# mit-acl/roman

Hardware: AMD Instinct MI355X
Metric: submap-pair alignments/sec + p50 latency at n=m=200 objects, d=512 (higher is better)
Workload: dtype f64 (fixed-point SpMV sums); 1 GPU; config 3: batch of 256 submap pairs per GPU, n=200 m=200 d=512, method=semanticgrav (xyz + 512-d descriptors + gravity prior); p50 latency measured on config 2 (single pair); pairs_per_call=256, n=200, m=200, d=512, method=semanticgrav, batches_in_flight=3

## Files before the change

roman_amd/csrc/kernels.hip.h:

```cpp
#pragma once
#include <hip/hip_cooperative_groups.h>
#include <hip/hip_runtime.h>
#include <stdint.h>
#include <type_traits>
#include "../../include/roman_hip.h"

namespace roman {

constexpr int WAVE = 64;
constexpr int STREAM_MAXL = 3072;

struct DevParams {
    roman_params_t p;
    double sig2;
    double sin_unc;
    double x_eps;
    double x_mindist;
    int32_t single;
    int32_t gravity;
    int32_t F;
    int32_t max_compact;
    int32_t gmode;
    int32_t diag_one;
    int32_t keep_all;
// ... 2266 lines not shown
        for (int t = 0; t < nw; ++t) { if (t < w) wbase += wsum[t]; tot += wsum[t]; }
        const uint32_t carry = carry_s;
        if (s < nsl) sliceBase[lo + s] = carry + wbase + inc - v;
        __syncthreads();
        if (tid == 0) carry_s = carry + tot;
        __syncthreads();
    }
    if (tid == 0) st[b].nnzCap = carry_s;
}

struct LivePools { int32_t* lp; int32_t* li; int32_t* lj; double* ls; double* ld; double* lza; double* lzb; };

__global__ void __launch_bounds__(1024) k_upper(const ProbDesc* __restrict__ probs, const ProbState* __restrict__ st,
                                                const BatchTotals* __restrict__ tot, const ItemDesc* __restrict__ items,
                                                const unsigned long long* __restrict__ maskPool,
                                                uint16_t* __restrict__ listPool, const uint32_t* __restrict__ listOff,
                                                uint32_t* __restrict__ rowCnt, const uint32_t* __restrict__ perm,
                                                const uint32_t* __restrict__ rowPos, LivePools src, LivePools dst, int RPB)
{
    __shared__ uint16_t posS[STREAM_MAXL + 64];
    const int tid = threadIdx.x, nt = blockDim.x, lane = tid & 63, w = tid >> 6, wpb = nt >> 6;
    const int nItems = tot->items;
    int staged = -1;
    const int Gx_ = (nItems + 7) >> 3;
    for (int sIdx_ = blockIdx.x; (sIdx_ >> 3) < Gx_; sIdx_ += gridDim.x) {
        const int t = (sIdx_ & 7) * Gx_ + (sIdx_ >> 3);
        if (t >= nItems) continue;
        const ItemDesc it = items[t];
        const int b = it.b;
        if (uni_i(st[b].kind) == 0) {
        const int L = st[b].L;
        const int W = (L + 63) >> 6;
        const int64_t lo = probs[b].liveOff, mo = st[b].maskOff;
        uint16_t* const lists = listPool + st[b].listOff;
        const int nrows = min(RPB, L - it.row0);
        if (staged != b) {
            __syncthreads();
            for (int q = tid; q < W * 64; q += nt) posS[q] = (q < L) ? (uint16_t)rowPos[lo + q] : (uint16_t)0;
            __syncthreads();
            staged = b;
        }
        const int RW = (nrows + wpb - 1) / wpb;
        const int r0 = w * RW, r1 = min(nrows, r0 + RW);
        if (r0 < r1) {
            const int p0 = it.row0 + r0;
            uint32_t glo = 0u, ghi = 0u;
            for (int wd = 0; wd < W; ++wd) {
                const unsigned long long gt = __ballot((int)posS[(wd << 6) + lane] > p0);
                writelane2(glo, ghi, gt, (uint32_t)__builtin_amdgcn_readfirstlane(wd));
            }
            unsigned long long behind = ((unsigned long long)ghi << 32) | glo;
            const int nr = r1 - r0;
            const int kv = (lane < nr) ? (int)perm[lo + p0 + lane] : 0;
            const uint32_t ov = (lane < nr) ? listOff[lo + p0 + lane] : 0u;
            if (lane < nr) { dst.lp[lo + p0 + lane] = src.lp[lo + kv]; dst.ld[lo + p0 + lane] = src.ld[lo + kv]; }
            unsigned long long m_n = (lane < W) ? maskPool[mo + (int64_t)__builtin_amdgcn_readlane(kv, 0) * W + lane] : 0ull;
            for (int i = 0; i < nr; ++i) {
                const int p = p0 + i;
                const unsigned long long raw = m_n;
                int kn = 0;
                if (i + 1 < nr) {
                    kn = __builtin_amdgcn_readlane(kv, i + 1);
                    m_n = (lane < W) ? maskPool[mo + (int64_t)kn * W + lane] : 0ull;
                }
                const unsigned long long mine = raw & behind;
                const uint32_t c = (uint32_t)__popcll(mine);
                const uint32_t ex = wave_excl_scan(c, lane);
                const uint32_t cnt = (uint32_t)__builtin_amdgcn_readlane((int)(ex + c), WAVE - 1);
                {
                    uint16_t* lst = lists + (uint32_t)__builtin_amdgcn_readlane((int)ov, i);
                    unsigned long long m = mine; uint32_t e = ex;
                    while (m) { lst[e++] = (uint16_t)((lane << 6) + __builtin_ctzll(m)); m &= m - 1ull; }
                    if (lane < 4 && cnt + (uint32_t)lane < ((cnt + 3u) & ~3u)) lst[cnt + lane] = (uint16_t)0xffffu;
                }
                if (lane == 0) rowCnt[lo + p] = cnt;
                if (i + 1 < nr && lane == (kn >> 6)) behind &= ~(1ull << (kn & 63));
            }
        }
        }
    }
}

constexpr int LISTS_NT = 1024;

__global__ void __launch_bounds__(LISTS_NT) k_lists(int B, const ProbDesc* __restrict__ probs, ProbState* __restrict__ st, BatchTotals* __restrict__ tot,
                                                   const unsigned long long* __restrict__ maskPool,
                                                   uint16_t* __restrict__ listPool, uint32_t* __restrict__ listOff,
                                                   uint32_t* __restrict__ rowCnt, uint32_t* __restrict__ perm, uint32_t* __restrict__ rowPos,
                                                   LivePools src, LivePools dst, long long capList,
                                                   int eqMax ,
                                                   int degGiven )
{
    __shared__ uint32_t degS[STREAM_MAXL + 64];
    __shared__ uint32_t keyS[4096];
    __shared__ unsigned long long tabS[STREAM_MAXL + 64];
    __shared__ uint16_t tmpS[STREAM_MAXL + 64];
    __shared__ uint32_t wsum[LISTS_NT / 64 + 4];
    __shared__ int okS;
    static_assert(STREAM_MAXL <= 4096, "sort capacity");
    const int tid = threadIdx.x, lane = tid & 63, w = tid >> 6;
    constexpr int NW = LISTS_NT / 64;
    const int g = lane >> 4, sl = lane & 15;
    for (int b = blockIdx.x; b < B; b += gridDim.x) {
        __syncthreads();
        if (st[b].kind != 0) continue;
        const int L = st[b].L;
        if (L <= 0) continue;
        const int W = (L + 63) >> 6;
        const int64_t lo = probs[b].liveOff, mo = st[b].maskOff;
        const unsigned long long* mrow = maskPool + mo;
        auto fetch = [&](int k0_, int c0_) -> unsigned long long {
            const int k = k0_ + g, c = c0_ + sl;
            const bool valid = k < L && c < W;
            unsigned long long m = mrow[(int64_t)min(k, L - 1) * W + min(c, W - 1)];
            if (!valid) m = 0ull;
            if (c == (k >> 6)) m &= ((k & 63) == 63) ? 0ull : (~0ull << ((k & 63) + 1));
            return m;
        };
        auto advance = [&](int& k0_, int& c0_) { c0_ += 16; if (c0_ >= W) { k0_ += 4 * NW; c0_ = k0_ >> 6; } };
        auto sweep = [&](auto f) {
            constexpr int PF = 6;
            int kr[PF], cr[PF]; unsigned long long mr[PF];
            int kn = 4 * w, cn = kn >> 6;
#pragma unroll
            for (int i = 0; i < PF; ++i) { kr[i] = kn; cr[i] = cn; mr[i] = fetch(kn, cn); advance(kn, cn); }
            while (kr[0] < L) {
#pragma unroll
                for (int i = 0; i < PF; ++i) {
                    const int kc = kr[i], cc = cr[i]; const unsigned long long mc = mr[i];
                    kr[i] = kn; cr[i] = cn; mr[i] = fetch(kn, cn); advance(kn, cn);
                    f(kc + g, mc, cc + sl);
                }
            }
        };
#ifdef ROMAN_LISTS_TIMING
        unsigned long long tl_[6]; tl_[0] = __builtin_readcyclecounter();
#define LMARK(i_) tl_[i_] = __builtin_readcyclecounter()
#else
#define LMARK(i_) do { } while (0)
#endif
        for (int q = tid; q < L; q += LISTS_NT) degS[q] = degGiven ? rowCnt[lo + q] : 0u;
        __syncthreads();
        if (!degGiven) {
        sweep([&](int k, unsigned long long m, int c) {
            if (m) {
                atomicAdd(&degS[k], (uint32_t)__popcll(m));
                while (m) { atomicAdd(&degS[(c << 6) + __builtin_ctzll(m)], 1u); m &= m - 1ull; }
            }
        });
        __syncthreads();
        }
        LMARK(1);
        int N = 64; while (N < L) N <<= 1;
        if (eqMax <= 0 || !place_keys(L, N, eqMax, [&](int k) { return degS[k]; }, keyS, reinterpret_cast<uint32_t*>(tabS), reinterpret_cast<uint32_t*>(tabS) + (STREAM_MAXL + 64), tmpS, wsum)) {
        for (int t = tid; t < N; t += LISTS_NT) keyS[t] = (t < L) ? (((degS[t] + 1u) << 12) | (uint32_t)(4095 - t)) : 0u;
        __syncthreads();
        for (int k2 = 2; k2 <= N; k2 <<= 1)
            for (int j2 = k2 >> 1; j2 > 0; j2 >>= 1) {
                for (int t = tid; t < (N >> 1); t += LISTS_NT) {
                    const int i1 = ((t & ~(j2 - 1)) << 1) | (t & (j2 - 1)), i2 = i1 | j2;
                    const uint32_t a = keyS[i1], c2 = keyS[i2];
                    const bool desc = (i1 & k2) == 0;
                    if ((a < c2) == desc) { keyS[i1] = c2; keyS[i2] = a; }
                }
                __syncthreads();
            }
        }
        LMARK(2);
        {
            const int PER = (L + LISTS_NT - 1) / LISTS_NT;
            uint32_t sum = 0;
            for (int t = 0; t < PER; ++t) {
                const int q = tid * PER + t;
                if (q < L) sum += (min((keyS[q] >> 12) - 1u, (uint32_t)(L - 1 - q)) + 3u) & ~3u;
            }
            const uint32_t inc = wave_incl_scan(sum);
            if (lane == WAVE - 1) wsum[w] = inc;
            __syncthreads();
            uint32_t wbase = 0, total = 0;
            for (int t = 0; t < NW; ++t) { if (t < w) wbase += wsum[t]; total += wsum[t]; }
            if (tid == 0) {
                const unsigned long long base = atomicAdd(&tot->listTop, (unsigned long long)total);
                st[b].listOff = (int64_t)base;
                const bool fits = (long long)(base + total) <= capList;
                if (!fits) { st[b].kind = 2; atomicAdd(&tot->overflow, 1); }
                okS = fits ? 1 : 0;
            }
            uint32_t run = wbase + inc - sum;
            for (int t = 0; t < PER; ++t) {
                const int q = tid * PER + t;
                if (q < L) {
                    const uint32_t k = 4095u - (keyS[q] & 4095u);
                    perm[lo + q] = k; rowPos[lo + k] = (uint32_t)q;
                    tabS[k] = ((unsigned long long)run << 16) | (unsigned long long)q; listOff[lo + q] = run; degS[k] = 0u;
                    run += (min((keyS[q] >> 12) - 1u, (uint32_t)(L - 1 - q)) + 3u) & ~3u;
                }
            }
        }
        __syncthreads();
        if (!okS) continue;
        uint16_t* const lists = listPool + st[b].listOff;
        LMARK(3);
        sweep([&](int k, unsigned long long m, int c) {
            if (!m) return;
            const unsigned long long tk = tabS[k];
            const uint32_t pk = (uint32_t)tk & 0xffffu, ok = (uint32_t)(tk >> 16);
            while (m) {
                const uint32_t q = (uint32_t)((c << 6) + __builtin_ctzll(m));
                m &= m - 1ull;
                const unsigned long long tq = tabS[q];
                const bool mine = pk < ((uint32_t)tq & 0xffffu);
                const uint32_t slot = atomicAdd(&degS[mine ? (uint32_t)k : q], 1u);
                lists[(mine ? ok : (uint32_t)(tq >> 16)) + slot] = (uint16_t)(mine ? q : (uint32_t)k);
            }
        });
        __syncthreads();
        LMARK(4);
        for (int p = tid; p < L; p += LISTS_NT) {
            const uint32_t k = 4095u - (keyS[p] & 4095u);
            const uint32_t cnt = degS[k];
            rowCnt[lo + p] = cnt;
            uint16_t* lst = lists + (uint32_t)(tabS[k] >> 16);
            for (uint32_t e = cnt; e < ((cnt + 3u) & ~3u); ++e) lst[e] = (uint16_t)0xffffu;
            dst.lp[lo + p] = src.lp[lo + k]; dst.ld[lo + p] = src.ld[lo + k];
        }
#ifdef ROMAN_LISTS_TIMING
        LMARK(5);
        if (tid == 0 && (b & 63) == 0) printf("[k_lists] b=%d L=%d cycles: degrees %llu sort %llu offsets %llu scatter %llu tail %llu\n", b, L,
                                              tl_[1] - tl_[0], tl_[2] - tl_[1], tl_[3] - tl_[2], tl_[4] - tl_[3], tl_[5] - tl_[4]);
#endif
#undef LMARK
    }
}

__global__ void __launch_bounds__(64) k_slicegeom(const ProbDesc* __restrict__ probs, ProbState* __restrict__ st,
                                                  const uint32_t* __restrict__ rowCnt,
                                                  uint32_t* __restrict__ sliceWidth, uint32_t* __restrict__ sliceBase)
{
    const int b = blockIdx.x, lane = threadIdx.x;
    if (st[b].kind != 0) return;
    const int L = st[b].L;
    const int64_t lo = probs[b].liveOff;
    const int nsl = (L + 63) >> 6;
    uint32_t width = 0;
    if (lane < nsl) {
        const int hi = min(L, (lane << 6) + 64);
        for (int p = lane << 6; p < hi; ++p) width = max(width, rowCnt[lo + p]);
        width = (width + 3u) & ~3u;
        sliceWidth[lo + lane] = width;
    }
    const uint32_t v = width * 64u;
    const uint32_t ex = wave_excl_scan(v, lane);
    if (lane < nsl) sliceBase[lo + lane] = ex;
    if (lane == WAVE - 1) st[b].nnzCap = ex + v;
}

__global__ void __launch_bounds__(1024) k_probscan(int B, int NG , long long capNnz, ProbState* __restrict__ st, BatchTotals* __restrict__ tot)
{
    __shared__ long long shl[17];
    __shared__ int shi[17];
    __shared__ int red[1];
    const int tid = threadIdx.x, nt = blockDim.x;
    const int PER = (B + nt - 1) / nt;
    const int b0 = tid * PER, b1 = min(B, b0 + PER);
    constexpr int PC = 8;
    int cK[PC], cL[PC]; uint32_t cC[PC];
#pragma unroll
    for (int j = 0; j < PC; ++j) { const int b = b0 + j; const bool in = j < PER && b < b1; cK[j] = in ? st[b].kind : 2; cL[j] = in ? st[b].L : 0; cC[j] = in ? st[b].nnzCap : 0u; }
    auto get = [&](int b, int& kind, int& L, long long& cap) {
        const int j = b - b0;
        if (j < PC) {
#pragma unroll
            for (int t = 0; t < PC; ++t) if (t == j) { kind = cK[t]; L = cL[t]; cap = (long long)cC[t]; }
        } else { kind = st[b].kind; L = st[b].L; cap = (long long)st[b].nnzCap; }
        if (kind >= 2) cap = 0;
    };
    long long sC = 0;
    for (int b = b0; b < b1; ++b) { int kind, L; long long cap; get(b, kind, L, cap); sC += cap; }
    long long totC; int totG;
    const long long baseC = block_excl_scan(sC, shl, totC);
    int sG = 0;
    {
        long long acc = baseC;
        for (int b = b0; b < b1; ++b) {
            int kind, L; long long cap; get(b, kind, L, cap);
            acc += cap;
            if (kind == 0 && acc <= capNnz) sG += min(NG, (L + 63) >> 6);
        }
    }
    const int baseG = block_excl_scan(sG, shi, totG);
    if (tid == 0) red[0] = 0;
    __syncthreads();
    int nover = 0;
    {
        long long acc = baseC; int gacc = baseG;
        for (int b = b0; b < b1; ++b) {
            int kind, L; long long cap; get(b, kind, L, cap);
            const bool fits = acc + cap <= capNnz;
            const int ng = (kind == 0 && fits) ? min(NG, (L + 63) >> 6) : 0;
            st[b].nnzOff = fits ? acc : 0; st[b].sgBase = gacc;
            if (!fits && kind < 2) { st[b].kind = 2; ++nover; }
            acc += cap; gacc += ng;
        }
    }
    for (int off = 32; off > 0; off >>= 1) nover += __shfl_xor(nover, off);
    if ((tid & 63) == 0 && nover) atomicAdd(&red[0], nover);
    __syncthreads();
// ... 3159 lines not shown
```

roman_amd/csrc/roman_hip.hip:

```cpp
#include <hip/hip_runtime.h>
#include <algorithm>
#include <cmath>
#include <cstdarg>
#include <cstdio>
#include <cstdlib>
#include <cstring>
#include <new>
#include <string>
#include <vector>

#include "kernels.hip.h"

using namespace roman;

namespace {

thread_local std::string g_last_error;

struct DevBuf {
    void* p = nullptr; size_t cap = 0;
    hipError_t ensure(size_t bytes) {
        if (bytes <= cap) return hipSuccess;
        if (p) { hipError_t e = hipFree(p); p = nullptr; cap = 0; if (e != hipSuccess) return e; }
        size_t want = bytes + bytes / 4 + 256;
// ... 202 lines not shown
}
struct StageTimer {
    roman_ctx* c; int s;
    StageTimer(roman_ctx* c_, int s_) : c(c_), s(s_) { if (c->profile) { prof_flush(c, c->cur, s); (void)hipEventRecord(WS.evA[s], WS.stream); } }
    void stop() { if (c->profile) { (void)hipEventRecord(WS.evB[s], WS.stream); WS.pending[s] = true; } }
};

int dbg_stage(roman_ctx* c, const char* what)
{
    static const bool dbg = getenv("ROMAN_DEBUG") != nullptr;
    if (!dbg) return ROMAN_OK;
    const hipError_t e = hipStreamSynchronize(WS.stream);
    fprintf(stderr, "[roman] %-14s %s\n", what, e == hipSuccess ? "ok" : hipGetErrorString(e));
    fflush(stderr);
    return e == hipSuccess ? ROMAN_OK : fail(c, ROMAN_E_HIP, "%s failed: %s", what, hipGetErrorString(e));
}
#define DBG(c, what) do { int rc_ = dbg_stage((c), (what)); if (rc_) return rc_; } while (0)

struct BatchIn {
    int32_t B; const double* feats; const int64_t* off1; const int32_t* n1; const int64_t* off2; const int32_t* n2;
    int32_t F; const int32_t* assoc; const int64_t* assoc_off;
};

struct Sizing {
    double sumA = 0, maxA = 0, maskBound = 0;
    int expectMaxL = 0;
    long long capMaskWords = 0, capNnz = 0, capList = 0;
};

void harvest_totals(roman_ctx* c, bool wait)
{
    for (int k = 0; k < ROMAN_MAX_PIPELINE; ++k) {
        roman_ctx::Workspace& W = c->ws[k];
        if (!W.totPending || !W.totEvent) continue;
        if (wait) { if (hipEventSynchronize(W.totEvent) != hipSuccess) { (void)hipGetLastError(); continue; } }
        else if (hipEventQuery(W.totEvent) != hipSuccess) { (void)hipGetLastError(); continue; }
        W.totPending = false;
        const BatchTotals& t = *W.pinnedTotals;
        c->skippedTotal += t.overflow;
        if (W.totEpoch != c->histEpoch) continue;
        roman_ctx::Hist& H = c->hist;
        if (W.totMaxA > 0) H.rMaxL = std::max(H.rMaxL, (double)t.maxL / W.totMaxA);
        if (W.totMaskBound > 0) H.rMask = std::max(H.rMask, (double)t.needMaskWords / W.totMaskBound);
        if (W.totSumA > 0) H.rNnz = std::max(H.rNnz, (double)t.needNnz / W.totSumA);
        if (W.totSumA > 0) H.rList = std::max(H.rList, (double)t.listTop / W.totSumA);
        if (t.minStreamL <= SMALL_MAXL) H.smallSeen = true;
        if (t.maxStreamL > SMALL_MAXL) H.largeSeen = true;
        if (t.nGeneral > 0) H.generalSeen = true;
        if (t.cosScreened > 0) { H.cosSeen = true; H.cosDenseFrac = (double)t.cosDense / t.cosScreened; }
        H.valid = true;
    }
}

void estimate_sizes(roman_ctx* c, const DevParams& D, const roman_params_t* params, int32_t F, const std::vector<ProbDesc>& hd, Sizing* S)
{
    roman_ctx::Hist& H = c->hist;
    if (!H.tagged || H.F != F || memcmp(&H.params, params, sizeof(roman_params_t)) != 0) {
        H = roman_ctx::Hist{}; H.params = *params; H.F = F; H.tagged = true;
        ++c->histEpoch;
    }
    harvest_totals(c, false);
    const bool prunes = D.single && !D.keep_all;
    double heurMask = 0, heurNnz = 0; int heurMaxL = 0;
    for (const ProbDesc& d : hd) {
        const double nA = d.nA;
        S->sumA += nA; S->maxA = std::max(S->maxA, nA); S->maskBound += nA * std::ceil(nA / 64.0);
        const double capL = prunes ? std::min(nA, std::max(4096.0, nA / 8.0)) : nA;
        heurMaxL = std::max(heurMaxL, (int)capL);
        heurMask += capL * std::ceil(capL / 64.0);
        heurNnz += capL * std::min(capL, 96.0);
    }
    if (H.valid) {
        S->expectMaxL = prunes ? (int)std::min(S->maxA, std::ceil(H.rMaxL * S->maxA * 1.15) + 64.0) : (int)S->maxA;
        S->capMaskWords = (long long)(prunes ? H.rMask * S->maskBound * 1.3 + 4096.0 : S->maskBound);
        S->capNnz = (long long)(H.rNnz * S->sumA * 1.3 + 65536.0);
        S->capList = (long long)(H.rList * S->sumA * 1.3 + 65536.0);
    } else {
        S->expectMaxL = heurMaxL; S->capMaskWords = (long long)heurMask; S->capNnz = (long long)heurNnz + 65536;
        S->capList = (long long)(2.5 * heurNnz) + 65536;
    }
    S->capMaskWords = std::max<long long>(S->capMaskWords, 64);
    const char* tcap = getenv("ROMAN_TEST_CAPNNZ");
    if (tcap && !H.valid) S->capNnz = atoll(tcap);
}

int may_fallback(const DevParams& D, const std::vector<ProbDesc>& hd);

struct BatchOut { int32_t kmax; int32_t* assoc_out; int32_t* n_assoc_out; double* T_out; int32_t* status_out; roman_stats_t* stats_out; };

int make_solve_out(roman_ctx* c, int B, int64_t sumA, const BatchOut& out, SolveOut* O)
{
    const size_t R1 = (size_t)std::max<int64_t>(sumA, 1);
    HIPCHK(c, WS.uOut.ensure(sizeof(double) * R1)); HIPCHK(c, WS.nodesOrig.ensure(sizeof(int32_t) * R1));
    HIPCHK(c, WS.nSel.ensure(sizeof(int32_t) * (size_t)B));
    O->assoc_out = out.assoc_out; O->n_assoc_out = out.n_assoc_out; O->T_out = out.T_out; O->status_out = out.status_out; O->stats_out = out.stats_out; O->kmax = out.kmax;
    O->nodesOrig = WS.nodesOrig.as<int32_t>(); O->nSel = WS.nSel.as<int32_t>(); O->uOut = WS.uOut.as<double>();
    O->dbg = nullptr;
    return ROMAN_OK;
}

static hipError_t launch_cos_flagged(roman_ctx* c, hipStream_t stream, const DevParams& D, int B, int maxN1, int maxN2, const ProbDesc* dP, const double* feats,
                                     double* cosPool, const int32_t* dense);
static hipError_t launch_cos_sel(roman_ctx* c, hipStream_t stream, const DevParams& D, int B, int maxN1, int maxN2, const ProbDesc* dP, const double* feats, double* cosPool,
                                 int32_t* dense, bool approx)
{
    hipError_t e = dyn_lds(c, reinterpret_cast<const void*>(k_cos_sel), (size_t)CSEL_LDS);
    if (e != hipSuccess) return e;
    const double thr = approx ? INFINITY : D.p.cosine_min - 0x1p-6;
    hipLaunchKernelGGL(k_cos_sel, dim3((unsigned)B), dim3(1024), (size_t)CSEL_LDS, stream, D, B, dP, feats, cosPool, dense, thr);
    e = hipGetLastError();
    if (e != hipSuccess) return e;
    return launch_cos_flagged(c, stream, D, B, maxN1, maxN2, dP, feats, cosPool, dense);
}
static hipError_t launch_cos_live(roman_ctx* c, hipStream_t stream, const DevParams& D, int B, int maxN1, int maxN2, const ProbDesc* dP, const double* feats, double* cosPool,
                                  int32_t* dense, ProbState* st, const LivePools& LP)
{
    hipError_t e = dyn_lds(c, reinterpret_cast<const void*>(k_cos_live), (size_t)CSEL_LDS);
    if (e != hipSuccess) return e;
    hipLaunchKernelGGL(k_cos_live, dim3((unsigned)B), dim3(1024), (size_t)CSEL_LDS, stream, D, B, dP, feats, dense, D.p.cosine_min - 0x1p-6,
                       st, LP.lp, LP.li, LP.lj, LP.ls, LP.ld, LP.lza, LP.lzb);
    e = hipGetLastError();
    if (e != hipSuccess) return e;
    return launch_cos_flagged(c, stream, D, B, maxN1, maxN2, dP, feats, cosPool, dense);
}
static hipError_t launch_cos_flagged(roman_ctx* c, hipStream_t stream, const DevParams& D, int B, int maxN1, int maxN2, const ProbDesc* dP, const double* feats,
                                     double* cosPool, const int32_t* dense)
{
    hipError_t e;
    constexpr int TD = 5;
    using CD = CosDeal<TD>;
    const int Gd = CD::tiles(maxN1) * CD::tiles(maxN2);
    e = dyn_lds(c, reinterpret_cast<const void*>(k_cos_deal<TD, 0>), (size_t)CD::LDS);
    if (e != hipSuccess) return e;
    hipLaunchKernelGGL((k_cos_deal<TD, 0>), dim3((unsigned)(B >= 8 ? Gd * ((B + 7) / 8) * 8 : Gd * B)), dim3(256), (size_t)CD::LDS, stream, D, B, Gd, dP, feats, cosPool, (const int32_t*)dense);
    return hipGetLastError();
}
static bool cos_sel_applies(const roman_ctx* c, const DevParams& D, int B, int maxN1, int maxN2, int64_t poolRows)
{
    if (!D.single || D.pruned || !(D.p.cosine_max > D.p.cosine_min) || !std::isfinite(D.p.cosine_min) || !std::isfinite(D.p.cosine_max)) return false;
    if (maxN1 > CSEL_MAXN || maxN2 > CSEL_MAXN || maxN1 <= 0 || maxN2 <= 0) return false;
    if (poolRows * (int64_t)D.F * 8 >= (1LL << 32)) return false;
    const char* env = getenv("ROMAN_COS_SEL");
    if (env && env[0]) return env[0] == '1';
    if (2 * B < c->num_cu || D.p.cos_feature_dim < 64 || std::max(maxN1, maxN2) < 64) return false;
    roman_ctx::Hist& H = const_cast<roman_ctx*>(c)->hist;
    if (H.cosSeen && H.cosDenseFrac > 0.25) {
        if (++H.cosSkipped < 64) return false;
        H.cosSkipped = 0;
    }
    return true;
}


static int sort_eq_max()
{
    const char* e = getenv("ROMAN_SORT_EQMAX");
    return (e && e[0]) ? std::max(0, atoi(e)) : 512;
}

static hipError_t launch_cos(roman_ctx* c, hipStream_t stream, const DevParams& D, int B, int maxN1, int maxN2, const ProbDesc* dP, const double* feats, double* cosPool)
{
    static const char* env = getenv("ROMAN_COS");
    const int mode = env ? atoi(env) : 16;
    static const char* waveEnv = getenv("ROMAN_COS_WAVE");
    {
        const char* dealEnv = getenv("ROMAN_COS_DEAL");
// ... 219 lines not shown
            for (int wp = PRE_WAVES; wp >= 8; wp -= 4) {
                const size_t need = (size_t)(tc + PRE_COLPAD + 4) * 4 + (size_t)wp * (size_t)count_pre_wave_bytes(preRow, tc);
                if (need <= c->lds_max) { preNR = PRE_NR; preWpb = wp; preTC = tc; preLds = need; break; }
            }
            if (wpbEnv && preNR) {
                preWpb = std::min(preWpb, wpb);
                preLds = (size_t)(preTC + PRE_COLPAD + 4) * 4 + (size_t)preWpb * (size_t)count_pre_wave_bytes(preRow, preTC);
            }
            if (preNR) {
                const char* objEnv = getenv("ROMAN_COUNT_OBJ");
                const int no = (std::max(maxN, 1) + 1) & ~1;
                const size_t objBytes = (size_t)2 * no * 32 + 16;
                if (objEnv && objEnv[0] == '1' && preLds + (size_t)preTC * 4 + objBytes <= c->lds_max) { preNO = no; preLds += objBytes; }
            }
        }
    }

    StageTimer t1(c, ROMAN_STAGE_COUNT_PASS);
    {
        static const char* fusedEnv = getenv("ROMAN_SMALL_FUSED");
        const bool want = smallOut != nullptr && !(fusedEnv && fusedEnv[0] == '0') && D.p.maxiniters >= 1 && D.p.maxlsiters >= 1 && maxTab > 0 &&
                          (c->hist.valid ? c->hist.smallSeen : maxA <= 16 * SMALL_MAXL);
        if (want) {
            SolveOut O;
            int rc = make_solve_out(c, B, sumA, *smallOut, &O);
            if (rc) return rc;
            HIPCHK(c, hipMemsetAsync(WS.queue.as<int>() + 8, 0, sizeof(int), WS.stream));
            const bool fast = D.single && (D.p.single_mode == ROMAN_SINGLE_BOTH || D.p.single_mode == ROMAN_SINGLE_OFFDIAG) && D.p.distance_weight == 1.0 &&
                              D.p.fusion_method != ROMAN_FUSE_ARITHMETIC_MEAN && D.p.fusion_method != ROMAN_FUSE_PRODUCT;
            constexpr size_t ldsSmall = small_lds_bytes();
            const int grid = std::max(1, std::min(B, c->num_cu * 12));
            auto ks = fast ? k_small<true> : k_small<false>;
            hipLaunchKernelGGL(ks, dim3(grid), dim3(64), ldsSmall, WS.stream, D, B, dP, dS, in.feats, in.assoc, WS.tabPool.as<double>(),
                               LP.lp, LP.li, LP.lj, LP.ls, LP.ld, LP.lza, LP.lzb, WS.plp.as<int32_t>(), WS.pld.as<double>(), WS.rowPos.as<uint32_t>(),
                               smallU0, O, WS.queue.as<int>() + 8);
    DBG(c, "k_small");
            static const char* onlyEnv = getenv("ROMAN_SMALL_ONLY");
            D.small_only = (c->hist.valid && !c->hist.generalSeen && !(onlyEnv && onlyEnv[0] == '0')) ? 1 : 0;
            Dout->small_only = D.small_only;
        }
    }
    hipLaunchKernelGGL(k_rowbase, dim3(1), dim3(B > 256 ? 1024 : 256), 0, WS.stream, B, RPB, SZ.capMaskWords, dS, dT, D.small_only, cosScreen ? (const int32_t*)WS.cosDense.as<int32_t>() : (const int32_t*)nullptr);
    DBG(c, "k_rowbase");
    if (!D.small_only) {
    hipLaunchKernelGGL(k_items, dim3(B), dim3(256), 0, WS.stream, RPB, dS, WS.items.as<ItemDesc>());
    DBG(c, "k_items");
    }
    if (sumA > 0 && !D.small_only) {
        const bool needTiled = D.allow_fallback || TCc < Lneed;
        int degGiven = 0;
        for (int tiled = 0; tiled < (needTiled ? 2 : 1); ++tiled) {
            const void* kc = nullptr;
#define ROMAN_KC(GM_) kc = tiled ? (NRc == 2 ? reinterpret_cast<const void*>(k_count<GM_, 2, true>) : reinterpret_cast<const void*>(k_count<GM_, 1, true>)) \
                                 : (NRc == 2 ? reinterpret_cast<const void*>(k_count<GM_, 2, false>) : reinterpret_cast<const void*>(k_count<GM_, 1, false>))
            switch (D.gmode) { case 1: ROMAN_KC(1); break; case 2: ROMAN_KC(2); break; case 3: ROMAN_KC(3); break; default: ROMAN_KC(0); break; }
#undef ROMAN_KC
            const bool usePre = !tiled && preNR > 0;
            if (usePre) {
#define ROMAN_KP(GM_) kc = reinterpret_cast<const void*>(k_count<GM_, 1, false, true>)
                switch (D.gmode) { case 1: ROMAN_KP(1); break; case 2: ROMAN_KP(2); break; case 3: ROMAN_KP(3); break; default: ROMAN_KP(0); break; }
#undef ROMAN_KP
            }
            const size_t ldsK = usePre ? preLds : pairLds;
            const int wpbK = usePre ? preWpb : wpb;
            const int gridK = usePre ? c->num_cu * std::max(1, std::min(2048 / (wpbK * 64), (int)(c->lds_max / ldsK))) : pairGrid;
            const char* wholeEnv = getenv("ROMAN_COUNT_WHOLE");
            const bool wholeP = usePre && (wholeEnv ? wholeEnv[0] != '0' : B >= c->num_cu) && preLds + (size_t)preTC * 4 <= c->lds_max;
            if (wholeP) degGiven = 1;
            HIPCHK(c, dyn_lds(c, kc, ldsK + (wholeP ? (size_t)preTC * 4 : 0)));
            DevParams a_D = D; const ProbDesc* a_dP = dP; const ProbState* a_dS = dS; const BatchTotals* a_dT = dT; const ItemDesc* a_items = WS.items.as<ItemDesc>();
            const double* a_tab = WS.tabPool.as<double>(); const int32_t* a_li = LP.li; const int32_t* a_lj = LP.lj; const double* a_za = LP.lza; const double* a_zb = LP.lzb;
            uint32_t* a_rc = WS.rowCnt.as<uint32_t>(); unsigned long long* a_mask = WS.maskPool.as<unsigned long long>(); uint32_t* a_pref = WS.prefPool.as<uint32_t>();
            int a_TC = usePre ? preTC : TCc, a_lpw = usePre ? preRow : ldsPerWave;
            int a_RPB = wholeP ? -B : RPB;
            const uint16_t* a_qtab = WS.qtabPool.as<uint16_t>();
            const double* a_feats = in.feats; int a_NO = usePre ? preNO : 0;
            void* args[] = {&a_D, &a_dP, &a_dS, &a_dT, &a_items, &a_tab, &a_li, &a_lj, &a_za, &a_zb, &a_rc, &a_mask, &a_pref, &a_TC, &a_lpw, &a_RPB, &a_qtab, &a_feats, &a_NO};
            HIPCHK(c, hipLaunchKernel(kc, dim3(gridK), dim3(wpbK * 64), args, ldsK + (wholeP ? (size_t)preTC * 4 : 0), WS.stream));
        }
    DBG(c, "k_count");
        const char* listsEnv = getenv("ROMAN_LISTS");
        const int fusedLists = listsEnv ? (listsEnv[0] == '0' ? 0 : 1) : (B >= std::max(8, c->num_cu / 8) ? 1 : 0);
        if (fusedLists) {
            const char* llEnv = getenv("ROMAN_LISTS_LDS");
            const size_t listsPad = llEnv ? (size_t)std::max(0, atoi(llEnv)) : 0;
            if (listsPad) HIPCHK(c, dyn_lds(c, reinterpret_cast<const void*>(k_lists), listsPad));
            hipLaunchKernelGGL(k_lists, dim3((unsigned)std::max(1, std::min(B, 2 * c->num_cu))), dim3(LISTS_NT), listsPad, WS.stream, B, dP, dS, dT,
                               WS.maskPool.as<unsigned long long>(), WS.listPool.as<uint16_t>(), WS.listOff.as<uint32_t>(),
                               WS.rowCnt.as<uint32_t>(), WS.perm.as<uint32_t>(), WS.rowPos.as<uint32_t>(), LP, PP, (long long)SZ.capList, sort_eq_max(), degGiven);
    DBG(c, "k_lists");
        }
        if (!fusedLists || D.allow_fallback) {
        {
            const int Wexp = (expL + 63) / 64;
            const int tasks = ((Wexp + 7) / 8) * ((std::max(Wexp - 1, 1) + 7) / 8);
            const int T = std::max(tasks, 1);
            hipLaunchKernelGGL(k_mirror, dim3((unsigned)(T * ((B + 7) / 8) * 8)), dim3(512), 0, WS.stream, B, T, dS, WS.maskPool.as<unsigned long long>(), fusedLists);
    DBG(c, "k_mirror");
        }
        hipLaunchKernelGGL(k_rowprefix, dim3(c->num_cu * 2), dim3(1024), 0, WS.stream, dP, dS, dT, WS.items.as<ItemDesc>(),
                           WS.maskPool.as<unsigned long long>(), WS.prefPool.as<uint32_t>(), WS.rowCnt.as<uint32_t>(), RPB, fusedLists);
    DBG(c, "k_rowprefix");
        int sortThr = 1024;
        if (!D.allow_fallback) { int N2 = 64; while (N2 < expL) N2 <<= 1; sortThr = std::max(64, std::min(1024, N2 / 2)); }
        hipLaunchKernelGGL(k_rowsort, dim3(B), dim3(sortThr), 0, WS.stream, dP, dS, dT, WS.rowCnt.as<uint32_t>(), WS.rowPos.as<uint32_t>(), WS.perm.as<uint32_t>(),
                           WS.sliceWidth.as<uint32_t>(), WS.sliceBase.as<uint32_t>(), WS.listOff.as<uint32_t>(), SZ.capList, fusedLists, sort_eq_max());
    DBG(c, "k_rowsort");
        if (!fusedLists) {
        const int upThr = expL <= 256 ? 256 : 1024;
        hipLaunchKernelGGL(k_upper, dim3(c->num_cu * 2 * (1024 / upThr)), dim3(upThr), 0, WS.stream, dP, dS, dT, WS.items.as<ItemDesc>(),
                           WS.maskPool.as<unsigned long long>(), WS.listPool.as<uint16_t>(), WS.listOff.as<uint32_t>(),
                           WS.rowCnt.as<uint32_t>(), WS.perm.as<uint32_t>(), WS.rowPos.as<uint32_t>(), LP, PP, RPB);
    DBG(c, "k_upper");
        }
        }
        hipLaunchKernelGGL(k_slicegeom, dim3(B), dim3(64), 0, WS.stream, dP, dS, WS.rowCnt.as<uint32_t>(), WS.sliceWidth.as<uint32_t>(), WS.sliceBase.as<uint32_t>());
    DBG(c, "k_slicegeom");
    }
    static const char* ngEnv = getenv("ROMAN_FILL_NG");
    int NG = (int)std::max<int64_t>(1, std::min<int64_t>(FILLS_MAXSPI, (3 * (int64_t)c->num_cu + B / 2) / std::max(B, 1)));
    {
        const int stride = std::max(1, (c->num_cu & ~7) / 8);
        auto gcd = [](int a, int b) { while (b) { const int t = a % b; a = b; b = t; } return a; };
        while (NG > 1 && gcd(stride % NG, NG) != 1) --NG;
    }
    if (ngEnv) NG = std::max(1, std::min(FILLS_MAXSPI, atoi(ngEnv)));
    const int Wmax = std::max(1, D.stream_maxL / 64);
    const int SPI = (Wmax + std::min(NG, Wmax) - 1) / std::min(NG, Wmax);
    if (!D.small_only) {
    hipLaunchKernelGGL(k_probscan, dim3(1), dim3(B > 256 ? 1024 : 256), 0, WS.stream, B, NG, SZ.capNnz, dS, dT);
    DBG(c, "k_probscan");
    }
    t1.stop();

    StageTimer t2(c, ROMAN_STAGE_FILL);
    if (sumA > 0 && !D.small_only) {
        const int colBytesF = D.gravity ? 32 : 16;
        const int TCs = D.stream_maxL;
        static const char* objEnv = getenv("ROMAN_FILL_OBJ");
        const int NO = (std::max(maxN, 1) + 1) & ~1;
        const size_t groupLds = sizeof(uint32_t) * (size_t)(3 * SPI * 64 + 2 * (SPI + 1) + 2);
        const bool obj = (objEnv ? atoi(objEnv) != 0 : true) && (size_t)TCs * (16 + 2) + (size_t)64 * NO + groupLds <= c->lds_max;
        const size_t sliceLds = obj ? (size_t)TCs * (16 + 2) + (size_t)64 * NO + groupLds : (size_t)TCs * (colBytesF + 2) + groupLds;
        if (sliceLds > c->lds_max) return fail(c, ROMAN_E_TOO_LARGE, "internal: stream column tile does not fit the LDS");
        const bool fast = D.single && (D.p.single_mode == ROMAN_SINGLE_BOTH || D.p.single_mode == ROMAN_SINGLE_OFFDIAG) && D.p.distance_weight == 1.0 &&
                          D.p.fusion_method != ROMAN_FUSE_ARITHMETIC_MEAN && D.p.fusion_method != ROMAN_FUSE_PRODUCT;
        auto kf = D.gravity ? (fast ? k_fill_list<true, true, false> : k_fill_list<true, false, false>) : (fast ? k_fill_list<false, true, false> : k_fill_list<false, false, false>);
        if (obj) kf = D.gravity ? (fast ? k_fill_list<true, true, true> : k_fill_list<true, false, true>) : (fast ? k_fill_list<false, true, true> : k_fill_list<false, false, true>);
        HIPCHK(c, dyn_lds(c, reinterpret_cast<const void*>(kf), sliceLds));
        const int fillThr = expL <= 256 ? 256 : 1024;
        const int fillWgs = std::max(1, std::min(1024 / fillThr, (int)(c->lds_max / sliceLds)));
        hipLaunchKernelGGL(kf, dim3((unsigned)((c->num_cu & ~7) * fillWgs)), dim3(fillThr), sliceLds, WS.stream,
                           D, B, dP, dS, dT, WS.tabPool.as<double>(), in.feats, NO, LP.li, LP.lj, LP.ls, LP.lza, LP.lzb,
                           WS.listPool.as<uint16_t>(), WS.listOff.as<uint32_t>(), WS.rowCnt.as<uint32_t>(), WS.perm.as<uint32_t>(), WS.rowPos.as<uint32_t>(),
                           WS.sliceWidth.as<uint32_t>(), WS.sliceBase.as<uint32_t>(), WS.cols16.as<uint16_t>(), WS.vals.as<double>(), TCs, NG, SPI);
    DBG(c, "k_fill_list");
        if (D.allow_fallback && (SZ.maxA > D.stream_maxL || D.p.maxiniters < 1 || D.p.maxlsiters < 1)) {
            const int colBytesG = D.gravity ? 40 : 24;
            const size_t ringLds = (size_t)16 * 3 * FILL_Q * sizeof(uint32_t) + (size_t)FILL_RPB * FILL_ROWBYTES;
            static_assert(FILL_RPB >= 128, "the work items of a batch are blocks of at most 128 rows");
            int TCf = (int)std::min<size_t>((c->lds_max - ringLds) / colBytesG, 32768) & ~63;
            TCf = std::min(TCf, std::max(64, (Lneed + 63) & ~63));
            const size_t fillLds = ringLds + (size_t)TCf * colBytesG;
            const int fillGrid = c->num_cu * std::max(1, std::min(2, (int)(c->lds_max / fillLds)));
            if (D.idx16) {
                auto kg = D.gravity ? k_fill<true, uint16_t, true> : k_fill<false, uint16_t, true>;
                HIPCHK(c, dyn_lds(c, reinterpret_cast<const void*>(kg), fillLds));
                hipLaunchKernelGGL(kg, dim3(fillGrid), dim3(1024), fillLds, WS.stream, D, dP, dS, dT, WS.items.as<ItemDesc>(), WS.tabPool.as<double>(),
                                   LP.li, LP.lj, LP.ls, LP.lza, LP.lzb,
                                   WS.rowCnt.as<uint32_t>(), WS.maskPool.as<unsigned long long>(), WS.prefPool.as<uint32_t>(), WS.rowPos.as<uint32_t>(),
                                   WS.sliceWidth.as<uint32_t>(), WS.sliceBase.as<uint32_t>(), WS.cols16.as<uint16_t>(), WS.vals.as<double>(), TCf, RPB, (const uint32_t*)WS.perm.as<uint32_t>());
            } else {
// ... 1258 lines not shown
```

Baseline: 173,200 alignments/s.

## Queue edge pairs per wave and stage list scatter in LDS window

Result: faster. 178,700 alignments/s, median of 6 (+3.1%).

```diff
diff --git a/roman_amd/csrc/kernels.hip.h b/roman_amd/csrc/kernels.hip.h
--- a/roman_amd/csrc/kernels.hip.h
+++ b/roman_amd/csrc/kernels.hip.h
@@ -2372,6 +2372,8 @@
 }
 
 constexpr int LISTS_NT = 1024;
+constexpr int LISTS_QRUN = 256;
+constexpr int LISTS_QCAP = 512;
 
 __global__ void __launch_bounds__(LISTS_NT) k_lists(int B, const ProbDesc* __restrict__ probs, ProbState* __restrict__ st, BatchTotals* __restrict__ tot,
                                                    const unsigned long long* __restrict__ maskPool,
@@ -2379,15 +2381,19 @@
                                                    uint32_t* __restrict__ rowCnt, uint32_t* __restrict__ perm, uint32_t* __restrict__ rowPos,
                                                    LivePools src, LivePools dst, long long capList,
                                                    int eqMax ,
-                                                   int degGiven )
-{
+                                                   int degGiven ,
+                                                   int winCap )
+{
+    extern __shared__ __attribute__((aligned(16))) uint16_t winS[];
     __shared__ uint32_t degS[STREAM_MAXL + 64];
-    __shared__ uint32_t keyS[4096];
+    __shared__ uint32_t keyS[(LISTS_NT / 64) * LISTS_QCAP];
     __shared__ unsigned long long tabS[STREAM_MAXL + 64];
     __shared__ uint16_t tmpS[STREAM_MAXL + 64];
     __shared__ uint32_t wsum[LISTS_NT / 64 + 4];
     __shared__ int okS;
     static_assert(STREAM_MAXL <= 4096, "sort capacity");
+    static_assert(LISTS_QRUN % 64 == 0 && LISTS_QCAP >= LISTS_QRUN + 64 && (LISTS_NT / 64) * LISTS_QCAP >= 4096, "k_lists queue");
+    uint32_t* const qS = keyS;
     const int tid = threadIdx.x, lane = tid & 63, w = tid >> 6;
     constexpr int NW = LISTS_NT / 64;
     const int g = lane >> 4, sl = lane & 15;
@@ -2457,6 +2463,7 @@
             }
         }
         LMARK(2);
+        uint32_t total = 0;
         {
             const int PER = (L + LISTS_NT - 1) / LISTS_NT;
             uint32_t sum = 0;
@@ -2467,7 +2474,7 @@
             const uint32_t inc = wave_incl_scan(sum);
             if (lane == WAVE - 1) wsum[w] = inc;
             __syncthreads();
-            uint32_t wbase = 0, total = 0;
+            uint32_t wbase = 0;
             for (int t = 0; t < NW; ++t) { if (t < w) wbase += wsum[t]; total += wsum[t]; }
             if (tid == 0) {
                 const unsigned long long base = atomicAdd(&tot->listTop, (unsigned long long)total);
@@ -2481,7 +2488,7 @@
                 const int q = tid * PER + t;
                 if (q < L) {
                     const uint32_t k = 4095u - (keyS[q] & 4095u);
-                    perm[lo + q] = k; rowPos[lo + k] = (uint32_t)q;
+                    perm[lo + q] = k; rowPos[lo + k] = (uint32_t)q; tmpS[q] = (uint16_t)k;
                     tabS[k] = ((unsigned long long)run << 16) | (unsigned long long)q; listOff[lo + q] = run; degS[k] = 0u;
                     run += (min((keyS[q] >> 12) - 1u, (uint32_t)(L - 1 - q)) + 3u) & ~3u;
                 }
@@ -2491,28 +2498,84 @@
         if (!okS) continue;
         uint16_t* const lists = listPool + st[b].listOff;
         LMARK(3);
+        {
+        uint32_t* const qw = qS + w * LISTS_QCAP;
+        uint32_t qn = 0;
+        auto lds_order = [&]() {
+            __builtin_amdgcn_fence(__ATOMIC_RELEASE, "wavefront"); __builtin_amdgcn_wave_barrier(); __builtin_amdgcn_fence(__ATOMIC_ACQUIRE, "wavefront");
+        };
+        auto place = [&](uint32_t base, uint32_t n, auto full) {
+            constexpr int CH = LISTS_QRUN / WAVE;
+            uint32_t kk[CH], qq[CH], slot[CH]; unsigned long long tk[CH], tq[CH]; bool act[CH];
+#pragma unroll
+            for (int x = 0; x < CH; ++x) {
+                const uint32_t idx = (uint32_t)(x * WAVE + lane);
+                act[x] = decltype(full)::value || idx < n;
+                const uint32_t e = qw[base + (act[x] ? idx : 0u)];
+                kk[x] = e >> 16; qq[x] = e & 0xffffu;
+                tk[x] = tabS[kk[x]]; tq[x] = tabS[qq[x]];
+            }
+#pragma unroll
+            for (int x = 0; x < CH; ++x) {
+                const bool mine = ((uint32_t)tk[x] & 0xffffu) < ((uint32_t)tq[x] & 0xffffu);
+                if (act[x]) slot[x] = atomicAdd(&degS[mine ? kk[x] : qq[x]], 1u);
+            }
+#pragma unroll
+            for (int x = 0; x < CH; ++x) {
+                const bool mine = ((uint32_t)tk[x] & 0xffffu) < ((uint32_t)tq[x] & 0xffffu);
+                const uint32_t at = (uint32_t)((mine ? tk[x] : tq[x]) >> 16) + slot[x];
+                const uint16_t v = (uint16_t)(mine ? qq[x] : kk[x]);
+                if (act[x]) { if (at < (uint32_t)winCap) winS[at] = v; else lists[at] = v; }
+            }
+        };
+        auto drain = [&]() {
+            if (qn >= (uint32_t)LISTS_QRUN) {
+                lds_order();
+                while (qn >= (uint32_t)LISTS_QRUN) { qn -= LISTS_QRUN; place(qn, LISTS_QRUN, std::true_type{}); }
+                lds_order();
+            }
+        };
         sweep([&](int k, unsigned long long m, int c) {
-            if (!m) return;
-            const unsigned long long tk = tabS[k];
-            const uint32_t pk = (uint32_t)tk & 0xffffu, ok = (uint32_t)(tk >> 16);
-            while (m) {
-                const uint32_t q = (uint32_t)((c << 6) + __builtin_ctzll(m));
-                m &= m - 1ull;
-                const unsigned long long tq = tabS[q];
-                const bool mine = pk < ((uint32_t)tq & 0xffffu);
-                const uint32_t slot = atomicAdd(&degS[mine ? (uint32_t)k : q], 1u);
-                lists[(mine ? ok : (uint32_t)(tq >> 16)) + slot] = (uint16_t)(mine ? q : (uint32_t)k);
-            }
+            const uint32_t cnt = (uint32_t)__popcll(m);
+            const uint32_t incl = wave_incl_scan(cnt);
+            const uint32_t npairs = (uint32_t)__builtin_amdgcn_readlane((int)incl, WAVE - 1);
+            const uint32_t kq = ((uint32_t)k << 16) | (uint32_t)(c << 6);
+            if (qn + npairs <= (uint32_t)LISTS_QCAP) {
+                uint32_t at = qn + incl - cnt;
+                while (m) { qw[at++] = kq + (uint32_t)__builtin_ctzll(m); m &= m - 1ull; }
+                qn += npairs;
+            } else {
+                while (true) {
+                    const unsigned long long bm = __ballot(m != 0ull);
+                    if (bm == 0ull) break;
+                    if (m) {
+                        qw[qn + __builtin_amdgcn_mbcnt_hi((uint32_t)(bm >> 32), __builtin_amdgcn_mbcnt_lo((uint32_t)bm, 0u))] = kq + (uint32_t)__builtin_ctzll(m);
+                        m &= m - 1ull;
+                    }
+                    qn += (uint32_t)__popcll(bm);
+                    drain();
+                }
+            }
+            drain();
         });
+        lds_order();
+        if (qn) place(0u, qn, std::false_type{});
+        }
         __syncthreads();
         LMARK(4);
         for (int p = tid; p < L; p += LISTS_NT) {
-            const uint32_t k = 4095u - (keyS[p] & 4095u);
+            const uint32_t k = tmpS[p];
             const uint32_t cnt = degS[k];
             rowCnt[lo + p] = cnt;
-            uint16_t* lst = lists + (uint32_t)(tabS[k] >> 16);
-            for (uint32_t e = cnt; e < ((cnt + 3u) & ~3u); ++e) lst[e] = (uint16_t)0xffffu;
+            const uint32_t o = (uint32_t)(tabS[k] >> 16);
+            for (uint32_t e = o + cnt; e < o + ((cnt + 3u) & ~3u); ++e) { if (e < (uint32_t)winCap) winS[e] = (uint16_t)0xffffu; else lists[e] = (uint16_t)0xffffu; }
             dst.lp[lo + p] = src.lp[lo + k]; dst.ld[lo + p] = src.ld[lo + k];
+        }
+        {
+            const uint32_t nq = min(total, (uint32_t)winCap) >> 2;
+            __syncthreads();
+            for (uint32_t i = (uint32_t)tid; i < nq; i += LISTS_NT)
+                reinterpret_cast<uint2*>(lists)[i] = reinterpret_cast<const uint2*>(winS)[i];
         }
 #ifdef ROMAN_LISTS_TIMING
         LMARK(5);
diff --git a/roman_amd/csrc/roman_hip.hip b/roman_amd/csrc/roman_hip.hip
--- a/roman_amd/csrc/roman_hip.hip
+++ b/roman_amd/csrc/roman_hip.hip
@@ -308,6 +308,8 @@
     S->capMaskWords = std::max<long long>(S->capMaskWords, 64);
     const char* tcap = getenv("ROMAN_TEST_CAPNNZ");
     if (tcap && !H.valid) S->capNnz = atoll(tcap);
+    const char* tlist = getenv("ROMAN_TEST_CAPLIST");
+    if (tlist && !H.valid) S->capList = atoll(tlist);
 }
 
 int may_fallback(const DevParams& D, const std::vector<ProbDesc>& hd);
@@ -693,12 +695,20 @@
         const char* listsEnv = getenv("ROMAN_LISTS");
         const int fusedLists = listsEnv ? (listsEnv[0] == '0' ? 0 : 1) : (B >= std::max(8, c->num_cu / 8) ? 1 : 0);
         if (fusedLists) {
+            static size_t listsStatic = 0;
+            if (listsStatic == 0) {
+                hipFuncAttributes fa;
+                HIPCHK(c, hipFuncGetAttributes(&fa, reinterpret_cast<const void*>(k_lists)));
+                listsStatic = std::max<size_t>(fa.sharedSizeBytes, 1);
+            }
             const char* llEnv = getenv("ROMAN_LISTS_LDS");
-            const size_t listsPad = llEnv ? (size_t)std::max(0, atoi(llEnv)) : 0;
-            if (listsPad) HIPCHK(c, dyn_lds(c, reinterpret_cast<const void*>(k_lists), listsPad));
-            hipLaunchKernelGGL(k_lists, dim3((unsigned)std::max(1, std::min(B, 2 * c->num_cu))), dim3(LISTS_NT), listsPad, WS.stream, B, dP, dS, dT,
+            const size_t room = c->lds_max > listsStatic ? c->lds_max - listsStatic : 0;
+            const size_t winBytes = std::min(room, llEnv ? (size_t)std::max(0, atoi(llEnv)) : room) & ~(size_t)15;
+            if (winBytes) HIPCHK(c, dyn_lds(c, reinterpret_cast<const void*>(k_lists), winBytes));
+            hipLaunchKernelGGL(k_lists, dim3((unsigned)std::max(1, std::min(B, 2 * c->num_cu))), dim3(LISTS_NT), winBytes, WS.stream, B, dP, dS, dT,
                                WS.maskPool.as<unsigned long long>(), WS.listPool.as<uint16_t>(), WS.listOff.as<uint32_t>(),
-                               WS.rowCnt.as<uint32_t>(), WS.perm.as<uint32_t>(), WS.rowPos.as<uint32_t>(), LP, PP, (long long)SZ.capList, sort_eq_max(), degGiven);
+                               WS.rowCnt.as<uint32_t>(), WS.perm.as<uint32_t>(), WS.rowPos.as<uint32_t>(), LP, PP, (long long)SZ.capList, sort_eq_max(), degGiven,
+                               (int)(winBytes / sizeof(uint16_t)));
     DBG(c, "k_lists");
         }
         if (!fusedLists || D.allow_fallback) {
```
